# boundless-xyz/boundless

Hardware: AMD Instinct MI355X
Metric: segment-proofs/sec @ 2^20 cycles (higher is better)
Workload: dtype u32 (BabyBear Montgomery)

## Files before the change

boundless_amd/csrc/circuit_dev.hpp:

```cpp
#pragma once
#include "circuit.hpp"
#include "fp.hpp"
#include "poseidon2_arith.hpp"

namespace bx {
inline namespace BX_MAD_FLAVOUR {

constexpr i64 FINAL_MAX = ((i64)(P / 2) - 1) * ((i64)1 << 32);
static_assert(ub(FINAL_MAX) < (i64)P && FINAL_MAX <= SREDC_MAX, "FINAL_MAX");

template <int V>
struct IntC {
    static constexpr int value = V;
};
template <int BEGIN, int END, class F>
BX_HD void static_for(F&& f) {
    if constexpr (BEGIN < END) {
        f(IntC<BEGIN>{});
        static_for<BEGIN + 1, END>(f);
    }
}

template <int TT, int GG>
struct ConsPlan {
    static constexpr int NPOOL = (int)Circuit::POOL;
    static constexpr i64 BC = (i64)(P / 2);
    static constexpr i64 chain_bound() {
        i64 y = BC;
        for (int f = 2; f + 1 < GG; ++f) y = ub(y * BC);
        return y;
    }
    static constexpr i64 TERM = chain_bound() * BC;
    static constexpr int ISZ = (int)(SREDC_MAX / TERM) < 4 ? (int)(SREDC_MAX / TERM) : 4;
    static_assert(ISZ >= 1 && ISZ * TERM <= SREDC_MAX, "cons_sum: inner group beyond sredc's range");

    int nq = 0, no = 0, n2 = 0;
    int first[TT]{}, len[TT]{}, term[TT][ISZ]{};
    int obeg[TT + 1]{}, lbeg[TT + 1]{};
    i64 max_inner = 0, max_outer = 0, max_l2 = 0, max_l3 = 0;

    constexpr ConsPlan() {
        for (int g = 0; g < TT; ++g)
            for (int a = 0; a < NPOOL; ++a) {
                int members[TT]{}, n = 0;
                for (int t = 0; t < TT; ++t)
                    if ((int)Circuit::pool_idx((unsigned)t, 0u) == a) members[n++] = t;
                const int groups = (n + ISZ - 1) / ISZ;
                if (g >= groups) continue;
                const int sz = n / groups + (g < n % groups ? 1 : 0), at = g * (n / groups) + (g < n % groups ? g : n % groups);
                first[nq] = a;
                len[nq] = sz;
                for (int k = 0; k < sz; ++k) term[nq][k] = members[at + k];
                if (sz * TERM > max_inner) max_inner = sz * TERM;
                ++nq;
            }
        i64 rb[TT + 1]{};
        i64 cur = 0;
        for (int q = 0; q < nq; ++q) {
            const i64 add = ub(len[q] * TERM) * BC;
            if (q > 0 && cur + add > SREDC_MAX) {
                rb[no++] = ub(cur);
                obeg[no] = q;
                cur = 0;
            }
            cur += add;
            if (cur > max_outer) max_outer = cur;
        }
        rb[no++] = ub(cur);
        obeg[no] = nq;
        cur = 0;
        for (int o = 0; o < no; ++o) {
            const i64 add = rb[o] * (i64)MONT_ONE;
            if (o > 0 && cur + add > FINAL_MAX) {
                max_l3 += ub(cur) * (i64)MONT_ONE;
                lbeg[++n2] = o;
                cur = 0;
            }
            cur += add;
            if (cur > max_l2) max_l2 = cur;
        }
        max_l3 += ub(cur) * (i64)MONT_ONE;
        lbeg[++n2] = no;
    }
};
template <int TT, int GG>
inline constexpr ConsPlan<TT, GG> cons_plan{};

template <int TT, int GG>
BX_HD uint32_t cons_sum(const uint32_t (&pool_u)[Circuit::POOL], uint32_t T, uint32_t G) {
    if constexpr (TT > 0 && GG >= 3) {
        constexpr int N2 = cons_plan<TT, GG>.n2;
        static_assert(cons_plan<TT, GG>.max_inner <= SREDC_MAX && cons_plan<TT, GG>.max_outer <= SREDC_MAX, "cons_sum: a group sum beyond sredc's range");
        static_assert(cons_plan<TT, GG>.max_l2 <= FINAL_MAX && cons_plan<TT, GG>.max_l3 <= FINAL_MAX, "cons_sum: term count beyond the three reduction levels");
        i32 pool[Circuit::POOL];
#pragma unroll
        for (unsigned i = 0; i < Circuit::POOL; ++i) pool[i] = fp_centre(pool_u[i]);
        i64 acc3 = 0;
        i32 result = 0;
        static_for<0, N2>([&](auto lc) {
            constexpr int l = decltype(lc)::value;
            i64 acc2 = 0;
            static_for<cons_plan<TT, GG>.lbeg[l], cons_plan<TT, GG>.lbeg[l + 1]>([&](auto oc) {
                constexpr int o = decltype(oc)::value;
                i64 outer = 0;
                static_for<cons_plan<TT, GG>.obeg[o], cons_plan<TT, GG>.obeg[o + 1]>([&](auto qc) {
                    constexpr int q = decltype(qc)::value;
                    i64 inner = 0;
                    static_for<0, cons_plan<TT, GG>.len[q]>([&](auto kc) {
                        constexpr int k = decltype(kc)::value;
                        constexpr unsigned t = (unsigned)cons_plan<TT, GG>.term[q][k];
                        i32 y = pool[Circuit::pool_idx(t, 1u)];
#pragma unroll
                        for (int f = 2; f + 1 < GG; ++f) y = sredc(smul(y, pool[Circuit::pool_idx(t, (unsigned)f)], f), f);
                        inner = smad(y, pool[Circuit::pool_idx(t, (unsigned)(GG - 1))], inner, k);
                    });
                    outer = smad(sredc(inner, 3), pool[cons_plan<TT, GG>.first[q]], outer, q);
                });
                acc2 = smad_k(sredc(outer, 1), MONT_ONE, acc2, o);
            });
            const i32 r2 = sredc(acc2, 2);
            if constexpr (N2 == 1) result = r2;
            else acc3 = smad_k(r2, MONT_ONE, acc3, l);
        });
        if constexpr (N2 > 1) result = sredc(acc3, 0);
        return (uint32_t)(result + (result < 0 ? (i32)P : 0));
    } else if constexpr (TT > 0) {
        static_assert(TT <= 3 * 8 * 7 && GG >= 1, "cons_sum: term count beyond the three reduction levels");
        i32 pool[Circuit::POOL];
#pragma unroll
        for (unsigned i = 0; i < Circuit::POOL; ++i) pool[i] = fp_centre(pool_u[i]);
        constexpr int GRP = 3, NG = (TT + GRP - 1) / GRP;
        i64 acc2 = 0, acc3 = 0;
        i32 result = 0;
#pragma unroll
        for (int g = 0; g < NG; ++g) {
            const int nk = (g + 1) * GRP <= TT ? GRP : TT - g * GRP;
            i64 acc = 0;
#pragma unroll
            for (int k = 0; k < GRP; ++k) {
                if (k < nk) {
                    const i32 x = pool[Circuit::pool_idx((unsigned)(g * GRP + k), 0u)];
                    if constexpr (GG == 1) acc = smad_k(x, MONT_ONE, acc, k);
                    else acc = smad(x, pool[Circuit::pool_idx((unsigned)(g * GRP + k), 1u)], acc, k);
                }
            }
            const i32 r = sredc(acc, 3);
            acc2 = smad_k(r, MONT_ONE, acc2, g);
            if ((g & 7) == 7 || g == NG - 1) {
                const i32 r2 = sredc(acc2, 1);
                acc2 = 0;
                if constexpr (NG <= 8) result = r2;
                else acc3 = smad_k(r2, MONT_ONE, acc3, 2);
            }
        }
        if constexpr (NG > 8) result = sredc(acc3, 0);
        return (uint32_t)(result + (result < 0 ? (i32)P : 0));
    } else {
        uint32_t sum = 0;
        for (uint32_t t = 0; t < T; ++t) {
            uint32_t prod = pool_u[Circuit::pool_idx(t, 0u)];
            for (uint32_t f = 1; f < G; ++f) prod = fp_mul(prod, pool_u[Circuit::pool_idx(t, f)]);
            sum = fp_add(sum, prod);
        }
        return sum;
    }
}

struct DerivedRegs {
    uint32_t ring[8], u[3], k[4];
    BX_HD void fill(uint32_t (&pool)[Circuit::POOL], uint32_t slot1) const {
        pool[0] = u[0]; pool[1] = slot1; pool[2] = u[1]; pool[3] = u[2];
#pragma unroll
        for (int q = 0; q < 8; ++q) pool[4 + q] = ring[q];
#pragma unroll
        for (int q = 0; q < 4; ++q) pool[12 + q] = k[q];
    }
    BX_HD void shift(uint32_t d, uint32_t next_u, uint32_t next_k) {
#pragma unroll
        for (int q = 7; q > 0; --q) ring[q] = ring[q - 1];
        ring[0] = d;
        u[0] = u[1]; u[1] = u[2]; u[2] = next_u;
        k[0] = k[1]; k[1] = k[2]; k[2] = k[3]; k[3] = next_k;
    }
};

}
}
```

Baseline: 28.53.

## Share pairwise products across degree-4 constraint terms via compile-time pair plan

Adds a compile-time PairPlan for degree-4 constraint sums that splits each four-factor term into two pool-pair products. It picks splits that maximise reuse of the same pair across terms, then orders terms so each shared pair is reduced once and consumed in groups of three per sredc. The aim is fewer Montgomery multiply/reduce operations than the previous per-term chained product. In exchange it adds a complex constexpr planner with compile-time cost, and may raise register pressure from live pair values.

```diff
diff --git a/boundless_amd/csrc/circuit_dev.hpp b/boundless_amd/csrc/circuit_dev.hpp
--- a/boundless_amd/csrc/circuit_dev.hpp
+++ b/boundless_amd/csrc/circuit_dev.hpp
@@ -86,9 +86,196 @@
 template <int TT, int GG>
 inline constexpr ConsPlan<TT, GG> cons_plan{};
 
+template <int TT>
+struct PairPlan {
+    static constexpr int NPOOL = (int)Circuit::POOL, NID = NPOOL * NPOOL;
+    static constexpr i64 BC = (i64)(P / 2);
+    static constexpr i64 PAIR = ub(BC * BC);
+    static constexpr i64 TERM = PAIR * PAIR;
+    static constexpr int GRP = (int)(SREDC_MAX / TERM);
+    static_assert(GRP == 3 && GRP * TERM <= SREDC_MAX, "cons_sum: pair group beyond sredc's range");
+    static constexpr int pair_id(unsigned a, unsigned b) { return a < b ? (int)(a * NPOOL + b) : (int)(b * NPOOL + a); }
+
+    int np = 0, ng = 0, n2 = 0;
+    int pa[2 * TT]{}, pb[2 * TT]{};
+    int seq[TT]{}, s1[TT]{}, s2[TT]{};
+    int pbeg[TT + 1]{};
+    int gbeg[TT + 1]{}, lbeg[TT + 1]{};
+    int max_live = 0;
+    i64 max_group = 0, max_l2 = 0, max_l3 = 0;
+
+    constexpr PairPlan() {
+        int sp[TT][3][2]{}, pop[NID]{}, ref[NID]{}, ch[TT]{};
+        for (int t = 0; t < TT; ++t) {
+            unsigned x[4]{};
+            for (unsigned f = 0; f < 4; ++f) x[f] = Circuit::pool_idx((unsigned)t, f);
+            for (int s = 0; s < 3; ++s) {
+                sp[t][s][0] = pair_id(x[0], x[s + 1]);
+                sp[t][s][1] = pair_id(x[s == 0 ? 2 : 1], x[s == 2 ? 2 : 3]);
+                ++pop[sp[t][s][0]];
+                ++pop[sp[t][s][1]];
+            }
+        }
+        for (int t = 0; t < TT; ++t) {
+            for (int s = 1; s < 3; ++s)
+                if (pop[sp[t][s][0]] + pop[sp[t][s][1]] > pop[sp[t][ch[t]][0]] + pop[sp[t][ch[t]][1]]) ch[t] = s;
+            ++ref[sp[t][ch[t]][0]];
+            ++ref[sp[t][ch[t]][1]];
+        }
+        for (int sweep = 0; sweep < 4; ++sweep)
+            for (int t = 0; t < TT; ++t) {
+                --ref[sp[t][ch[t]][0]];
+                --ref[sp[t][ch[t]][1]];
+                int best = 0, best_new = 3, best_ref = 0;
+                for (int s = 0; s < 3; ++s) {
+                    const int a = sp[t][s][0], b = sp[t][s][1];
+                    const int fresh = (ref[a] == 0) + (ref[b] == 0 && b != a), shared = ref[a] + ref[b];
+                    if (fresh < best_new || (fresh == best_new && shared > best_ref)) best = s, best_new = fresh, best_ref = shared;
+                }
+                ch[t] = best;
+                ++ref[sp[t][best][0]];
+                ++ref[sp[t][best][1]];
+            }
+        for (int pass = 0; pass < 2; ++pass) {
+            int snap[NID]{};
+            for (int i = 0; i < NID; ++i) snap[i] = ref[i];
+            for (int r = 1; r <= 4; ++r)
+                for (int p = 0; p < NID; ++p) {
+                    if (snap[p] != r || ref[p] == 0 || ref[p] > 4) continue;
+                    int users[4]{}, was[4]{}, nu = 0, moved = 0, delta = 0;
+                    for (int t = 0; t < TT; ++t)
+                        if (sp[t][ch[t]][0] == p || sp[t][ch[t]][1] == p) users[nu++] = t;
+                    for (int u = 0; u < nu; ++u) {
+                        was[u] = ch[users[u]];
+                        for (int k = 0; k < 2; ++k) delta -= (--ref[sp[users[u]][was[u]][k]] == 0);
+                    }
+                    for (; moved < nu; ++moved) {
+                        const int t = users[moved];
+                        int best = -1, best_new = 3, best_ref = 0;
+                        for (int s = 0; s < 3; ++s) {
+                            const int a = sp[t][s][0], b = sp[t][s][1];
+                            if (a == p || b == p) continue;
+                            const int fresh = (ref[a] == 0) + (ref[b] == 0 && b != a), shared = ref[a] + ref[b];
+                            if (best < 0 || fresh < best_new || (fresh == best_new && shared > best_ref)) best = s, best_new = fresh, best_ref = shared;
+                        }
+                        if (best < 0) break;
+                        ch[t] = best;
+                        for (int k = 0; k < 2; ++k) delta += (ref[sp[t][best][k]]++ == 0);
+                    }
+                    if (moved < nu || delta > 0 || (delta == 0 && pass == 0)) {
+                        for (int u = 0; u < moved; ++u)
+                            for (int k = 0; k < 2; ++k) --ref[sp[users[u]][ch[users[u]]][k]];
+                        for (int u = 0; u < nu; ++u) {
+                            ch[users[u]] = was[u];
+                            for (int k = 0; k < 2; ++k) ++ref[sp[users[u]][was[u]][k]];
+                        }
+                    }
+                }
+        }
+        int num[NID]{}, live = 0, glen = 0, gp[2 * GRP]{};
+        bool placed[TT]{};
+        for (int i = 0; i < NID; ++i) num[i] = -1;
+        for (int slot = 0; slot < TT;) {
+            int best = -1, best_new = 3, best_last = -1;
+            if (glen < GRP)
+                for (int t = 0; t < TT; ++t) {
+                    if (placed[t]) continue;
+                    const int a = sp[t][ch[t]][0], b = sp[t][ch[t]][1];
+                    bool clash = false;
+                    for (int k = 0; k < 2 * glen; ++k) clash = clash || gp[k] == a || gp[k] == b;
+                    if (clash) continue;
+                    const int fresh = (num[a] < 0) + (num[b] < 0 && b != a);
+                    const int last = a == b ? (ref[a] == 2) : (ref[a] == 1) + (ref[b] == 1);
+                    if (fresh < best_new || (fresh == best_new && last > best_last)) best = t, best_new = fresh, best_last = last;
+                }
+            if (best < 0) {
+                gbeg[++ng] = slot;
+                glen = 0;
+                continue;
+            }
+            const int a = sp[best][ch[best]][0], b = sp[best][ch[best]][1];
+            for (int k = 0; k < 2; ++k) {
+                const int id = k ? b : a;
+                if (num[id] < 0) {
+                    num[id] = np;
+                    pa[np] = id / NPOOL;
+                    pb[np] = id % NPOOL;
+                    ++np;
+                    ++live;
+                }
+            }
+            if (live > max_live) max_live = live;
+            live -= (--ref[a] == 0);
+            live -= (--ref[b] == 0);
+            placed[best] = true;
+            seq[slot] = best;
+            s1[slot] = num[a];
+            s2[slot] = num[b];
+            gp[2 * glen] = a;
+            gp[2 * glen + 1] = b;
+            ++glen;
+            pbeg[++slot] = np;
+        }
+        gbeg[++ng] = TT;
+        i64 cur = 0;
+        for (int g = 0; g < ng; ++g) {
+            const i64 sum = (gbeg[g + 1] - gbeg[g]) * TERM, add = ub(sum) * (i64)MONT_ONE;
+            if (sum > max_group) max_group = sum;
+            if (g > 0 && cur + add > FINAL_MAX) {
+                max_l3 += ub(cur) * (i64)MONT_ONE;
+                lbeg[++n2] = g;
+                cur = 0;
+            }
+            cur += add;
+            if (cur > max_l2) max_l2 = cur;
+        }
+        max_l3 += ub(cur) * (i64)MONT_ONE;
+        lbeg[++n2] = ng;
+    }
+};
+template <int TT>
+inline constexpr PairPlan<TT> pair_plan{};
+
 template <int TT, int GG>
 BX_HD uint32_t cons_sum(const uint32_t (&pool_u)[Circuit::POOL], uint32_t T, uint32_t G) {
-    if constexpr (TT > 0 && GG >= 3) {
+    if constexpr (TT > 0 && GG == 4) {
+        constexpr int N2 = pair_plan<TT>.n2;
+        static_assert(pair_plan<TT>.max_group <= SREDC_MAX, "cons_sum: a group sum beyond sredc's range");
+        static_assert(pair_plan<TT>.max_l2 <= FINAL_MAX && pair_plan<TT>.max_l3 <= FINAL_MAX, "cons_sum: term count beyond the three reduction levels");
+        i32 pool[Circuit::POOL];
+#pragma unroll
+        for (unsigned i = 0; i < Circuit::POOL; ++i) pool[i] = fp_centre(pool_u[i]);
+        i32 pr[pair_plan<TT>.np];
+        i64 acc3 = 0;
+        i32 result = 0;
+        static_for<0, N2>([&](auto lc) {
+            constexpr int l = decltype(lc)::value;
+            i64 acc2 = 0;
+            static_for<pair_plan<TT>.lbeg[l], pair_plan<TT>.lbeg[l + 1]>([&](auto gc) {
+                constexpr int g = decltype(gc)::value;
+                i64 acc = 0;
+                static_for<pair_plan<TT>.gbeg[g], pair_plan<TT>.gbeg[g + 1]>([&](auto sc) {
+                    constexpr int s = decltype(sc)::value;
+                    static_for<pair_plan<TT>.pbeg[s], pair_plan<TT>.pbeg[s + 1]>([&](auto pc) {
+                        constexpr int p = decltype(pc)::value;
+                        pr[p] = sredc(smul(pool[pair_plan<TT>.pa[p]], pool[pair_plan<TT>.pb[p]], p), p);
+                        BX_ASSERT_BOUND(pr[p] <= PairPlan<TT>::PAIR && pr[p] >= -PairPlan<TT>::PAIR, "cons_sum pair");
+                    });
+                    acc = smad(pr[pair_plan<TT>.s1[s]], pr[pair_plan<TT>.s2[s]], acc, s);
+                });
+                acc2 = smad_k(sredc(acc, 3), MONT_ONE, acc2, g);
+            });
+            BX_ASSERT_BOUND(acc2 <= FINAL_MAX && acc2 >= -FINAL_MAX, "cons_sum second level");
+            const i32 r2 = sredc(acc2, 2);
+            if constexpr (N2 == 1) result = r2;
+            else acc3 = smad_k(r2, MONT_ONE, acc3, l);
+        });
+        if constexpr (N2 > 1) {
+            BX_ASSERT_BOUND(acc3 <= FINAL_MAX && acc3 >= -FINAL_MAX, "cons_sum third level");
+            result = sredc(acc3, 0);
+        }
+        return (uint32_t)(result + (result < 0 ? (i32)P : 0));
+    } else if constexpr (TT > 0 && GG >= 3) {
         constexpr int N2 = cons_plan<TT, GG>.n2;
         static_assert(cons_plan<TT, GG>.max_inner <= SREDC_MAX && cons_plan<TT, GG>.max_outer <= SREDC_MAX, "cons_sum: a group sum beyond sredc's range");
         static_assert(cons_plan<TT, GG>.max_l2 <= FINAL_MAX && cons_plan<TT, GG>.max_l3 <= FINAL_MAX, "cons_sum: term count beyond the three reduction levels");
```

Result: faster. 29.92 (median of 6 runs) (+4.9%).
